# talmolab/track-mjx

Measured on AMD Instinct MI355X. Metric: env-steps/sec (whole node), rodent task @ 4096 envs/GPU, higher is better.
Workload: dtype f32

## Files before the change

### track_mjx_amd/csrc/wave_physics.h

```cpp
#pragma once
#include "tm_common.h"
#include "wave_layout.h"

#ifdef TM_HOST_EMU
#define TMW_NL 64
#define TMW_FOR for (int lane = 0; lane < 64; lane++)
#define TMW_SYNC() do { } while (0)
#define TMW_LI lane
#define TMW_LANE_DECL
#else
#define TMW_NL 1
#define TMW_FOR if (true)
#ifdef TMW_HARD_SYNC
#define TMW_SYNC() __syncthreads()
#else
#define TMW_SYNC() do { __builtin_amdgcn_fence(__ATOMIC_RELEASE, "wavefront"); __builtin_amdgcn_wave_barrier(); __builtin_amdgcn_fence(__ATOMIC_ACQUIRE, "wavefront"); } while (0)
#endif
#define TMW_LI 0
#define TMW_LANE_DECL const int lane = c.lane;
#endif
#define TMW_REG(type, name) type name[TMW_NL]
#ifdef TM_HOST_EMU
#define TMW_DUP_LANES_OK 0
#else
// ... 806 lines not shown
#pragma unroll
      for (int u = 0; u < 8; u++) {
        int mc = m0 + u < 64 ? m0 + u : 63;
        lm[u] = tmw_readlane(x, mc);
        ab[u] = tm_f2i(tmw_readlane(arow, mc));
      }
      TMW_FOR {
        float v[8]; int ad[8];
#pragma unroll
        for (int u = 0; u < 8; u++) ad[u] = lane > m0 + u ? ab[u] + lane : K.l_dummy + lane;
#pragma unroll
        for (int u = 0; u < 8; u++) v[u] = L[ad[u]];
        float s = acc[TMW_LI];
#pragma unroll
        for (int u = 0; u < 8; u++) s += lane > m0 + u ? lm[u] * v[u] : 0.f;
        acc[TMW_LI] = s;
      }
    }
    TMW_FOR { if (lane >= 1 && lane <= d) L[K.l_LD + ak + lane] = -acc[TMW_LI]; }
    TMW_SYNC();
  }
}
#define TMW_RL 63
TM_DEV float tmw_rcp(float x) {
#ifdef TM_HOST_EMU
  return 1.f / x;
#else
  float r = __builtin_amdgcn_rcpf(x);
  return fmaf(fmaf(-x, r, 1.f), r, r);
#endif
}
#ifdef TM_HOST_EMU
#define TMW_MASK(m64) (((((unsigned long long)(m64)) >> lane) & 1ull) != 0ull)
#define TMW_SCHED_FENCE() do { } while (0)
#define TMW_PIN(x) do { } while (0)
#else
TM_DEV unsigned long long tmw_lit64(unsigned long long m64) {
  unsigned hi = (unsigned)(m64 >> 32);
  asm("" : "+s"(hi));
  return ((unsigned long long)hi << 32) | (unsigned)m64;
}
#define TMW_MASK(m64) __builtin_amdgcn_inverse_ballot_w64((((unsigned long long)(m64)) >> 31) == 0x1ffffffffull ? tmw_lit64((unsigned long long)(m64)) : (unsigned long long)(m64))
#define TMW_PIN(x) asm volatile("" : "+v"(x))
#define TMW_SCHED_FENCE() __builtin_amdgcn_sched_barrier(0)
#endif
#define TMW_M_LT(n) ((n) >= 64 ? ~0ull : ((1ull << (n)) - 1ull))
#define TMW_M_EQ(n) (1ull << (n))
#define TMW_M_RANGE(a, b) (TMW_M_LT(b) & ~TMW_M_LT(a))
#ifdef TM_HOST_EMU
struct tmw_f2 { float x, y; };
TM_DEV tmw_f2 tmw_fnma2(float ax, float ay, float bx, float by, tmw_f2 c) { tmw_f2 r; r.x = c.x - ax * bx; r.y = c.y - ay * by; return r; }
#define TMW_PIN2(v) do { } while (0)
#else
typedef float tmw_f2 __attribute__((ext_vector_type(2)));
TM_DEV tmw_f2 tmw_fnma2(float ax, float ay, float bx, float by, tmw_f2 c) { tmw_f2 a = {ax, ay}, b = {bx, by}; return __builtin_elementwise_fma(-a, b, c); }
#define TMW_PIN2(v) asm volatile("" : "+v"(v))
#endif
#define TMW_ROW(arr, k) (((k) & 1) ? arr[(k) >> 1][TMW_LI].y : arr[(k) >> 1][TMW_LI].x)
#define TMW_SET_ROW(arr, k, v) do { if ((k) & 1) arr[(k) >> 1][TMW_LI].y = (v); else arr[(k) >> 1][TMW_LI].x = (v); } while (0)
template <typename F>
TM_DEV void tmw_rank1_rows(tmw_f2 (*T)[TMW_NL], const int CNT, const int BASE, const float *rs, const float *rk, F after_top) {
  const int top = (CNT - 1) / 2;
  float alo = tmw_readlane(rs, BASE + 2 * top), ahi = 2 * top + 1 < CNT ? tmw_readlane(rs, BASE + 2 * top + 1) : 0.f;
#pragma unroll
  for (int p = top; p >= 0; p--) {
    float nlo = 0.f, nhi = 0.f;
    if (p > 0) { nlo = tmw_readlane(rs, BASE + 2 * p - 2); nhi = tmw_readlane(rs, BASE + 2 * p - 1); }
    if (2 * p + 1 < CNT) {
      TMW_FOR { T[p][TMW_LI] = tmw_fnma2(alo, ahi, rk[TMW_LI], rk[TMW_LI], T[p][TMW_LI]); TMW_PIN2(T[p][TMW_LI]); }
    } else {
      TMW_FOR { T[p][TMW_LI].x -= alo * rk[TMW_LI]; TMW_PIN2(T[p][TMW_LI]); }
    }
    if (p == top) after_top();
    alo = nlo; ahi = nhi;
  }
}
template <int FIRST, int N, int D0, bool EULER, bool RHS = EULER>
TM_DEV void tmw_rows_load(WCtx &c, const WLayout &K, tmw_f2 (*r)[TMW_NL], float hdamp, int rhs) {
  TmwModel &m = *c.mp; float *L = c.L; TMW_LANE_DECL
  const int adr0 = K.l_M + tmw_chain_madr(FIRST);
  TMW_REG(float, hd);
  if (EULER) { TMW_FOR { bool mine = TMW_MASK(TMW_M_RANGE(D0, D0 + N)); hd[TMW_LI] = mine ? L[K.l_hdamp + (mine ? FIRST + lane - D0 : 0)] : 0.f; } }
  TMW_FOR {
#pragma unroll
    for (int k = 0; k < N; k++) {
      const int dk = D0 + k, off = k * D0 + k * (k - 1) / 2 + k;
      float v = L[adr0 - lane + (off + dk)];
      if (EULER) v += TMW_MASK(TMW_M_EQ(dk)) ? hd[TMW_LI] : 0.f;
      v = TMW_MASK(TMW_M_LT(dk + 1)) ? v : 0.f;
      TMW_SET_ROW(r, k, v);
    }
    if (N & 1) r[N >> 1][TMW_LI].y = 0.f;
  }
  if (RHS) {
    TMW_REG(float, rhsv);
    TMW_FOR { rhsv[TMW_LI] = L[rhs + FIRST + (lane < N ? lane : N - 1)]; }
#pragma unroll
    for (int k = 0; k < N; k++) {
      float sk = tmw_readlane(rhsv, k);
      TMW_FOR { if (TMW_MASK(TMW_M_EQ(TMW_RL))) TMW_SET_ROW(r, k, sk); }
    }
  }
}
#ifdef TMW_TRUNK_F32
typedef float tmw_acc_t;
#else
typedef double tmw_acc_t;
#endif
struct TmwSchur {
#ifdef TM_HOST_EMU
  tmw_acc_t C[16][16];
#elif defined(TMW_TRUNK_F32)
  float __attribute__((ext_vector_type(4))) c;
#else
  double __attribute__((ext_vector_type(4))) c;
#endif
  float qa[4][TMW_NL], qb[4][TMW_NL];
  float yt[TMW_NL];
};
#ifndef TM_HOST_EMU
TM_DEV float tmw_pack4(float x0, float x1, float x2, float x3) {
  auto s01 = __builtin_amdgcn_permlane16_swap(tm_f2i(x0), tm_f2i(x1), false, false);
  auto s23 = __builtin_amdgcn_permlane16_swap(tm_f2i(x2), tm_f2i(x3), false, false);
  auto p = __builtin_amdgcn_permlane32_swap(s01[0], s23[0], false, false);
  return tm_i2f(p[0]);
}
TM_DEV int tmw_row_to0(int x, const int blk) {
  if (blk == 1) return __builtin_amdgcn_permlane16_swap(x, 0, false, false)[1];
  if (blk >= 2) {
    x = __builtin_amdgcn_permlane32_swap(x, 0, false, false)[1];
    if (blk == 3) x = __builtin_amdgcn_permlane16_swap(x, 0, false, false)[1];
  }
  return x;
}
TM_DEV double tmw_row_to0_d(double x, const int blk) {
  long long b; __builtin_memcpy(&b, &x, 8);
  int lo = tmw_row_to0((int)(b & 0xffffffffll), blk), hi = tmw_row_to0((int)(b >> 32), blk);
  b = ((long long)hi << 32) | (unsigned)lo;
  __builtin_memcpy(&x, &b, 8);
  return x;
}
TM_DEV double tmw_readlane_d(const double *v, int src) {
  long long b; __builtin_memcpy(&b, v, 8);
  int lo = __builtin_amdgcn_readlane((int)(b & 0xffffffffll), src), hi = __builtin_amdgcn_readlane((int)(b >> 32), src);
  b = ((long long)hi << 32) | (unsigned)lo;
  double r; __builtin_memcpy(&r, &b, 8);
  return r;
}
TM_DEV double tmw_rcp_d(double x) { double r = (double)__builtin_amdgcn_rcpf((float)x); return __builtin_fma(__builtin_fma(-x, r, 1.0), r, r); }
#else
TM_DEV double tmw_readlane_d(const double *v, int src) { return v[src]; }
TM_DEV double tmw_rcp_d(double x) { return 1.0 / x; }
#endif
#ifdef TMW_TRUNK_F32
TM_DEV float tmw_acc_readlane(const float *v, int src) { return tmw_readlane(v, src); }
TM_DEV float tmw_acc_rcp(float x) { return tmw_rcp(x); }
TM_DEV float tmw_acc_fnma(float a, float b, float c) { return fmaf(-a, b, c); }
#else
TM_DEV double tmw_acc_readlane(const double *v, int src) { return tmw_readlane_d(v, src); }
TM_DEV double tmw_acc_rcp(double x) { return tmw_rcp_d(x); }
TM_DEV double tmw_acc_fnma(double a, double b, double c) { return __builtin_fma(-a, b, c); }
TM_DEV float tmw_acc_readlane(const float *v, int src) { return tmw_readlane(v, src); }
TM_DEV float tmw_acc_rcp(float x) { return tmw_rcp(x); }
TM_DEV float tmw_acc_fnma(float a, float b, float c) { return fmaf(-a, b, c); }
#endif
template <bool EULER>
TM_DEV void tmw_schur_init(WCtx &c, const WLayout &K, TmwSchur &S, tmw_f2 (*tr)[TMW_NL], int rhs) {
  float *L = c.L; TMW_LANE_DECL
#ifdef TM_HOST_EMU
  for (int i = 0; i < 16; i++) for (int j = 0; j < 16; j++) S.C[i][j] = (i < TMW_RODENT_TRUNK) ? -(tmw_acc_t)((i & 1) ? tr[i >> 1][j].y : tr[i >> 1][j].x) : (tmw_acc_t)0;
  for (int q = 0; q < 4; q++) for (int l = 0; l < 64; l++) S.qa[q][l] = S.qb[q][l] = 0.f;
#else
#define TMW_TRROW(i) ((i) < TMW_RODENT_TRUNK ? -(((i) & 1) ? tr[(i) >> 1][0].y : tr[(i) >> 1][0].x) : 0.f)
#ifdef TMW_TRUNK_F32
  S.c[0] = tmw_pack4(TMW_TRROW(0), TMW_TRROW(4), TMW_TRROW(8), TMW_TRROW(12));
  S.c[1] = tmw_pack4(TMW_TRROW(1), TMW_TRROW(5), TMW_TRROW(9), TMW_TRROW(13));
  S.c[2] = tmw_pack4(TMW_TRROW(2), TMW_TRROW(6), TMW_TRROW(10), TMW_TRROW(14));
  S.c[3] = tmw_pack4(TMW_TRROW(3), TMW_TRROW(7), TMW_TRROW(11), TMW_TRROW(15));
#else
  S.c[0] = (double)tmw_pack4(TMW_TRROW(0), TMW_TRROW(1), TMW_TRROW(2), TMW_TRROW(3));
  S.c[1] = (double)tmw_pack4(TMW_TRROW(4), TMW_TRROW(5), TMW_TRROW(6), TMW_TRROW(7));
  S.c[2] = (double)tmw_pack4(TMW_TRROW(8), TMW_TRROW(9), TMW_TRROW(10), TMW_TRROW(11));
  S.c[3] = 0.0;
#endif
#undef TMW_TRROW
  for (int q = 0; q < 4; q++) S.qa[q][0] = S.qb[q][0] = 0.f;
#endif
  TMW_FOR { S.yt[TMW_LI] = EULER ? -L[rhs + (lane < TMW_RODENT_TRUNK ? lane : 0)] : 0.f; }
}
TM_DEV void tmw_schur_flush(TmwSchur &S) {
#ifdef TM_HOST_EMU
  for (int q = 0; q < 4; q++) for (int i = 0; i < 16; i++) for (int j = 0; j < 16; j++) S.C[i][j] += (tmw_acc_t)S.qa[q][i] * (tmw_acc_t)S.qb[q][j];
  for (int q = 0; q < 4; q++) for (int l = 0; l < 64; l++) S.qa[q][l] = S.qb[q][l] = 0.f;
#else
  float A = tmw_pack4(S.qa[0][0], S.qa[1][0], S.qa[2][0], S.qa[3][0]), B = tmw_pack4(S.qb[0][0], S.qb[1][0], S.qb[2][0], S.qb[3][0]);
#ifdef TMW_TRUNK_F32
  S.c = __builtin_amdgcn_mfma_f32_16x16x4f32(A, B, S.c, 0, 0, 0);
#else
  S.c = __builtin_amdgcn_mfma_f64_16x16x4f64((double)A, (double)B, S.c, 0, 0, 0);
#endif
  for (int q = 0; q < 4; q++) S.qa[q][0] = S.qb[q][0] = 0.f;
#endif
}
template <bool EULER>
TM_DEV void tmw_schur_apply(WCtx &c, TmwSchur &S, tmw_acc_t (*t)[TMW_NL]) {
  TMW_LANE_DECL
#pragma unroll
  for (int i = 0; i < TMW_RODENT_TRUNK; i++) {
#ifdef TM_HOST_EMU
    TMW_FOR { tmw_acc_t v = 0; if (lane < 16) v = -S.C[i][lane]; if (EULER && lane == TMW_RL) v = -(tmw_acc_t)S.yt[i]; t[i][TMW_LI] = v; }
#else
#ifdef TMW_TRUNK_F32
    float x = tm_i2f(tmw_row_to0(tm_f2i(S.c[i & 3]), i / 4));
#else
    double x = tmw_row_to0_d(S.c[i / 4], i & 3);
#endif
    tmw_acc_t v = TMW_MASK(TMW_M_LT(16)) ? -x : (tmw_acc_t)0;
    if (EULER) { float y = tmw_readlane(S.yt, i); v = TMW_MASK(TMW_M_EQ(TMW_RL)) ? (tmw_acc_t)(-y) : v; }
    t[i][0] = v;
#endif
  }
}
template <bool EULER, typename AT>
TM_DEV void tmw_trunk_factor(WCtx &c, const WLayout &K, AT (*t)[TMW_NL], int rhs) {
  float *L = c.L; TMW_LANE_DECL
  constexpr int N = TMW_RODENT_TRUNK;
  TMW_REG(float, dv); TMW_REG(float, yv);
  AT rs[2][TMW_NL], inv[2];
  TMW_FOR { dv[TMW_LI] = 0.f; yv[TMW_LI] = 0.f; }
  inv[(N - 1) & 1] = tmw_acc_rcp(tmw_acc_readlane(t[N - 1], N - 1));
  TMW_FOR { rs[(N - 1) & 1][TMW_LI] = t[N - 1][TMW_LI] * inv[(N - 1) & 1]; }
#pragma unroll
  for (int k = N - 1; k >= 0; k--) {
    const int off = k * (k - 1) / 2 + k, b = k & 1;
    if (k > 0) {
      { const AT a = tmw_acc_readlane(rs[b], k - 1); TMW_FOR { t[k - 1][TMW_LI] = tmw_acc_fnma(a, t[k][TMW_LI], t[k - 1][TMW_LI]); } }
      inv[b ^ 1] = tmw_acc_rcp(tmw_acc_readlane(t[k - 1], k - 1));
      TMW_FOR { rs[b ^ 1][TMW_LI] = t[k - 1][TMW_LI] * inv[b ^ 1]; }
    }
#pragma unroll
    for (int i = k - 2; i >= 0; i--) { const AT a = tmw_acc_readlane(rs[b], i); TMW_FOR { t[i][TMW_LI] = tmw_acc_fnma(a, t[k][TMW_LI], t[i][TMW_LI]); } }
    float yk = 0.f;
    if (EULER) yk = (float)tmw_acc_readlane(t[k], TMW_RL);
    TMW_FOR {
      if (EULER) yv[TMW_LI] = TMW_MASK(TMW_M_EQ(k)) ? yk : yv[TMW_LI];
      if (k > 0 && TMW_MASK(TMW_M_LT(k))) L[K.l_LD - lane + (off + k)] = (float)rs[b][TMW_LI];
      dv[TMW_LI] = TMW_MASK(TMW_M_EQ(k)) ? (float)inv[b] : dv[TMW_LI];
    }
  }
  TMW_FOR {
    if (TMW_MASK(TMW_M_LT(N))) { L[K.l_Dinv + lane] = dv[TMW_LI]; if (EULER) L[rhs + lane] = yv[TMW_LI]; }
  }
}

template <int FIRST, int N, int D0, bool EULER>
TM_DEV void tmw_rows_factor(WCtx &c, const WLayout &K, tmw_f2 (*r)[TMW_NL], TmwSchur *S, int rhs) {
  float *L = c.L; TMW_LANE_DECL
  const int adr0 = K.l_LD + tmw_chain_madr(FIRST);
  constexpr int Q0 = D0 > 0 ? tmw_chain_rows_before(FIRST) : 0;
  float rs[2][TMW_NL], rk[2][TMW_NL], inv[2];
  TMW_REG(float, dv);
  TMW_REG(float, yv);
  TMW_FOR { yv[TMW_LI] = 0.f; rk[(N - 1) & 1][TMW_LI] = TMW_ROW(r, N - 1); }
  inv[(N - 1) & 1] = tmw_rcp(tmw_readlane(rk[(N - 1) & 1], D0 + N - 1));
  TMW_FOR { rs[(N - 1) & 1][TMW_LI] = rk[(N - 1) & 1][TMW_LI] * inv[(N - 1) & 1]; }
#pragma unroll
  for (int k = N - 1; k >= 0; k--) {
    const int dk = D0 + k, off = k * D0 + k * (k - 1) / 2 + k, b = k & 1;
    if (k > 0) {
      tmw_rank1_rows(r, k, D0, rs[b], rk[b], [&]() {
        TMW_FOR { rk[b ^ 1][TMW_LI] = TMW_ROW(r, k - 1); }
        inv[b ^ 1] = tmw_rcp(tmw_readlane(rk[b ^ 1], dk - 1));
        TMW_FOR { rs[b ^ 1][TMW_LI] = rk[b ^ 1][TMW_LI] * inv[b ^ 1]; TMW_PIN(rs[b ^ 1][TMW_LI]); }
      });
    }
    float yk = 0.f;
    if (EULER) { yk = tmw_readlane(rk[b], TMW_RL); TMW_FOR { yv[TMW_LI] = TMW_MASK(TMW_M_EQ(k)) ? yk : yv[TMW_LI]; } }
    if (D0 > 0) {
      const int slot = (Q0 + (N - 1 - k)) & 3;
      TMW_FOR {
        float a = D0 < 16 ? (TMW_MASK(TMW_M_LT(D0)) ? rs[b][TMW_LI] : 0.f) : rs[b][TMW_LI];
        S->qa[slot][TMW_LI] = a;
        S->qb[slot][TMW_LI] = D0 < 16 ? (TMW_MASK(TMW_M_LT(D0)) ? rk[b][TMW_LI] : 0.f) : rk[b][TMW_LI];
      }
      if (EULER) { TMW_FOR { S->yt[TMW_LI] += S->qa[slot][TMW_LI] * yk; } }
      if (slot == 3) tmw_schur_flush(*S);
    }
    TMW_FOR {
      if (dk > 0 && TMW_MASK(TMW_M_LT(dk))) L[adr0 - lane + (off + dk)] = rs[b][TMW_LI];
      dv[TMW_LI] = TMW_MASK(TMW_M_EQ(dk)) ? inv[b] : dv[TMW_LI];
    }
  }
  TMW_FOR {
    if (TMW_MASK(TMW_M_RANGE(D0, D0 + N))) L[K.l_Dinv + FIRST - D0 + lane] = dv[TMW_LI];
    if (EULER && TMW_MASK(TMW_M_LT(N))) L[rhs + FIRST + lane] = yv[TMW_LI];
  }
}
template <int FIRST, int N, int D0, bool EULER>
TM_DEV void tmw_chain_factor(WCtx &c, const WLayout &K, TmwSchur *S, float hdamp, int rhs) {
  tmw_f2 r[(N + 1) / 2][TMW_NL];
  tmw_rows_load<FIRST, N, D0, EULER>(c, K, r, hdamp, rhs);
  tmw_rows_factor<FIRST, N, D0, EULER>(c, K, r, S, rhs);
}
template <bool EULER>
TM_DEV void tmw_factor_chains(WCtx &c, const WLayout &K, float hdamp, int rhs) {
  TmwSchur S;
  {
    tmw_f2 tr[(TMW_RODENT_TRUNK + 1) / 2][TMW_NL];
    tmw_rows_load<0, TMW_RODENT_TRUNK, 0, EULER, false>(c, K, tr, hdamp, rhs);
    tmw_schur_init<EULER>(c, K, S, tr, rhs);
  }
#define TMW_X(first, n, d0) tmw_chain_factor<first, n, d0, EULER>(c, K, &S, hdamp, rhs);
  TMW_RODENT_LEAF_CHAINS(TMW_X)
#undef TMW_X
  tmw_schur_flush(S);
  tmw_acc_t t[TMW_RODENT_TRUNK][TMW_NL];
  tmw_schur_apply<EULER>(c, S, t);
#if defined(TMW_TRUNK_ELIM_F32) && !defined(TMW_TRUNK_F32)
  { float tf[TMW_RODENT_TRUNK][TMW_NL];
    TMW_FOR { for (int i = 0; i < TMW_RODENT_TRUNK; i++) tf[i][TMW_LI] = (float)t[i][TMW_LI]; }
    tmw_trunk_factor<EULER, float>(c, K, tf, rhs); }
#else
  tmw_trunk_factor<EULER, tmw_acc_t>(c, K, t, rhs);
#endif
  TMW_SYNC();
}
TM_DEV void tmw_rows_accum(tmw_f2 &acc, const tmw_f2 (*S)[TMW_NL], const int CNT, const int BASE, const float *l, int li) {
#pragma unroll
  for (int p = 0; 2 * p < CNT; p++) {
    float alo = tmw_readlane(l, BASE + 2 * p), ahi = 2 * p + 1 < CNT ? tmw_readlane(l, BASE + 2 * p + 1) : 0.f;
    acc = tmw_fnma2(alo, ahi, S[p][li].x, S[p][li].y, acc);
  }
}
template <int FIRST, int N, int D0>
TM_DEV void tmw_chain_trunk_products(WCtx &c, const WLayout &K, const float (*Bp)[TMW_NL], const tmw_f2 (*tn)[TMW_NL], float (*P)[TMW_NL]) {
  float *L = c.L; TMW_LANE_DECL
  const int adr0 = K.l_LD + tmw_chain_madr(FIRST);
#ifdef TM_HOST_EMU
  (void)Bp;
  for (int k = 0; k < N; k++)
    TMW_FOR {
      float s = 0.f;
      if (lane < D0) for (int j = 0; j < D0; j++) s += L[adr0 + k * D0 + k * (k - 1) / 2 + k + (D0 + k) - j] * ((j & 1) ? tn[j >> 1][lane].y : tn[j >> 1][lane].x);
      P[k][TMW_LI] = s;
    }
#else
  (void)tn;
  typedef float __attribute__((ext_vector_type(4))) f4;
#pragma unroll
  for (int k0 = 0; k0 < N; k0 += 16) {
    const int kq = k0 + (lane & 15), kk = lane >> 4;
    const bool rowok = kq < N;
    const int kc = rowok ? kq : N - 1;
    const int base = adr0 + kc * D0 + kc * (kc - 1) / 2 + kc + (D0 + kc) - kk;
    f4 acc = {0.f, 0.f, 0.f, 0.f};
#pragma unroll
    for (int m = 0; 4 * m < D0; m++) {
      float a = L[base - 4 * m];
      a = (rowok && 4 * m + kk < D0) ? a : 0.f;
      acc = __builtin_amdgcn_mfma_f32_16x16x4f32(a, Bp[m][0], acc, 0, 0, 0);
    }
#pragma unroll
    for (int i = 0; i < 16; i++) {
      if (k0 + i >= N) break;
      float x = acc[i & 3];
      if ((i >> 2) == 1) x = tm_i2f(__builtin_amdgcn_permlane16_swap(tm_f2i(x), 0, false, false)[1]);
      else if ((i >> 2) >= 2) {
        x = tm_i2f(__builtin_amdgcn_permlane32_swap(tm_f2i(x), 0, false, false)[1]);
        if ((i >> 2) == 3) x = tm_i2f(__builtin_amdgcn_permlane16_swap(tm_f2i(x), 0, false, false)[1]);
      }
      P[k0 + i][0] = TMW_MASK(TMW_M_LT(D0)) ? x : 0.f;
    }
  }
#endif
}
template <int FIRST, int N, int D0>
TM_DEV void tmw_rows_invert(WCtx &c, const WLayout &K, tmw_f2 (*n)[TMW_NL], tmw_f2 (*tn)[TMW_NL], const float (*Bp)[TMW_NL]) {
  float *L = c.L; TMW_LANE_DECL
  const int adr0 = K.l_LD + tmw_chain_madr(FIRST);
  float l[N][TMW_NL], P[D0 > 0 ? N : 1][TMW_NL];
  tmw_f2 acc[TMW_NL];
  TMW_FOR {
#pragma unroll
    for (int k = 0; k < N; k++) {
      const int dk = D0 + k, off = k * D0 + k * (k - 1) / 2 + k;
      float v = L[adr0 - lane + (off + dk)];
      l[k][TMW_LI] = TMW_MASK(TMW_M_LT(dk)) ? v : 0.f;
    }
#pragma unroll
    for (int p = 0; p < (N + 1) / 2; p++) { n[p][TMW_LI].x = 0.f; n[p][TMW_LI].y = 0.f; }
  }
  if (D0 > 0) tmw_chain_trunk_products<FIRST, N, D0>(c, K, Bp, tn, P);
#pragma unroll
  for (int k = 0; k < N; k++) {
    const int dk = D0 + k, off = k * D0 + k * (k - 1) / 2 + k;
    TMW_FOR { acc[TMW_LI].x = (TMW_MASK(TMW_M_EQ(dk)) ? 1.f : 0.f) - (D0 > 0 ? P[D0 > 0 ? k : 0][TMW_LI] : 0.f); acc[TMW_LI].y = 0.f; }
    if (k > 0) { TMW_FOR { tmw_rows_accum(acc[TMW_LI], n, k, D0, l[k], TMW_LI); } }
    TMW_FOR {
      float v = acc[TMW_LI].x + acc[TMW_LI].y;
      TMW_SET_ROW(n, k, v);
      if (TMW_MASK(TMW_M_LT(dk + 1))) L[adr0 - lane + (off + dk)] = v;
    }
  }
}
template <int FIRST, int N, int D0>
TM_DEV void tmw_chain_invert(WCtx &c, const WLayout &K, tmw_f2 (*tn)[TMW_NL], const float (*Bp)[TMW_NL]) {
  tmw_f2 n[(N + 1) / 2][TMW_NL];
  tmw_rows_invert<FIRST, N, D0>(c, K, n, tn, Bp);
}
TM_DEV void tmw_invert_chains(WCtx &c, const WLayout &K) {
  tmw_f2 tn[(TMW_RODENT_TRUNK + 1) / 2][TMW_NL];
  float Bp[(TMW_RODENT_TRUNK + 3) / 4][TMW_NL];
  tmw_rows_invert<0, TMW_RODENT_TRUNK, 0>(c, K, tn, tn, Bp);
#ifndef TM_HOST_EMU
#define TMW_TN(i) ((i) < TMW_RODENT_TRUNK ? (((i) & 1) ? tn[(i) >> 1][0].y : tn[(i) >> 1][0].x) : 0.f)
#pragma unroll
  for (int m = 0; m < (TMW_RODENT_TRUNK + 3) / 4; m++) Bp[m][0] = tmw_pack4(TMW_TN(4 * m), TMW_TN(4 * m + 1), TMW_TN(4 * m + 2), TMW_TN(4 * m + 3));
#undef TMW_TN
#endif
#define TMW_X(first, n, d0) tmw_chain_invert<first, n, d0>(c, K, tn, Bp);
  TMW_RODENT_LEAF_CHAINS(TMW_X)
#undef TMW_X
  TMW_SYNC();
}
template <int FIRST, int N, int D0>
TM_DEV void tmw_rows_subst(WCtx &c, const WLayout &K, const float *xt, float *z, int x) {
  float *L = c.L; TMW_LANE_DECL
  constexpr int QMAX = D0 + N - 1;
  TMW_REG(float, bv);
  TMW_FOR {
    int k = lane < N ? lane : N - 1;
    int base = K.l_LD + tmw_chain_madr(FIRST) + k * D0 + k * (k - 1) / 2 + k + D0 + k - QMAX;
    bv[TMW_LI] = tm_i2f(base);
    z[TMW_LI] = L[x + FIRST + k] * L[K.l_Dinv + FIRST + k];
  }
#pragma unroll
  for (int q = 0; q < D0; q++) {
    float xq = tmw_readlane(xt, q);
    TMW_FOR { z[TMW_LI] -= L[tm_f2i(bv[TMW_LI]) + (QMAX - q)] * xq; }
  }
#pragma unroll
  for (int q = D0; q < QMAX; q++) {
    float xq = tmw_readlane(z, q - D0);
    TMW_FOR { float v = L[tm_f2i(bv[TMW_LI]) + (QMAX - q)]; z[TMW_LI] = TMW_MASK(TMW_M_RANGE(q - D0 + 1, N)) ? z[TMW_LI] - v * xq : z[TMW_LI]; }
  }
  TMW_FOR { if (TMW_MASK(TMW_M_LT(N))) L[x + FIRST + lane] = z[TMW_LI]; }
}
TM_DEV void tmw_subst_chains(WCtx &c, const WLayout &K, int x) {
  TMW_LANE_DECL
  TMW_REG(float, xt); TMW_REG(float, z);
  TMW_FOR { xt[TMW_LI] = 0.f; }
  tmw_rows_subst<0, TMW_RODENT_TRUNK, 0>(c, K, xt, xt, x);
#define TMW_X(first, n, d0) tmw_rows_subst<first, n, d0>(c, K, xt, z, x);
  TMW_RODENT_LEAF_CHAINS(TMW_X)
#undef TMW_X
  TMW_SYNC();
}
template <int FIRST, int N, int D0>
TM_DEV void tmw_rows_colacc(WCtx &c, const WLayout &K, int A, const float *xv, float *acc) {
  float *L = c.L; TMW_LANE_DECL
  const int adr0 = A + tmw_chain_madr(FIRST);
#pragma unroll
  for (int k = N - 1; k >= 1 - (D0 > 0); k--) {
    const int dk = D0 + k, off = k * D0 + k * (k - 1) / 2 + k;
    float xk = tmw_readlane(xv, dk);
    TMW_FOR { float v = L[adr0 - lane + (off + dk)]; acc[TMW_LI] += (TMW_MASK(TMW_M_LT(dk)) ? v : 0.f) * xk; }
  }
}
template <bool SOLVE>
TM_DEV void tmw_colpart_chains(WCtx &c, const WLayout &K, int A, int x, int out) {
  float *L = c.L; TMW_LANE_DECL
  float xv[TMW_RODENT_NCHAIN + 1][TMW_NL], acc[TMW_RODENT_NCHAIN + 1][TMW_NL];
  { int ci = 0;
#define TMW_X(first, n, d0) TMW_FOR { bool mine = TMW_MASK(TMW_M_RANGE(d0, d0 + n)); xv[ci][TMW_LI] = mine ? L[x + (mine ? first - d0 + lane : 0)] : 0.f; acc[ci][TMW_LI] = 0.f; } ci++;
  TMW_RODENT_LEAF_CHAINS(TMW_X)
  TMW_X(0, TMW_RODENT_TRUNK, 0)
#undef TMW_X
  }
  { int ci = 0;
#define TMW_X(first, n, d0) tmw_rows_colacc<first, n, d0>(c, K, A, xv[ci], acc[ci]); TMW_FOR { acc[TMW_RODENT_NCHAIN][TMW_LI] += TMW_MASK(TMW_M_LT(d0)) ? acc[ci][TMW_LI] : 0.f; } ci++;
  TMW_RODENT_LEAF_CHAINS(TMW_X)
#undef TMW_X
  tmw_rows_colacc<0, TMW_RODENT_TRUNK, 0>(c, K, A, xv[ci], acc[ci]); }
  { int ci = 0;
#define TMW_STORE(first, n, d0) TMW_FOR { if (TMW_MASK(TMW_M_RANGE(d0, d0 + n))) { float v = acc[ci][TMW_LI]; if (SOLVE) v = (xv[ci][TMW_LI] + v) * L[K.l_Dinv + first - d0 + lane]; L[out + first - d0 + lane] = v; } } ci++;
  TMW_RODENT_LEAF_CHAINS(TMW_STORE)
  TMW_STORE(0, TMW_RODENT_TRUNK, 0)
#undef TMW_STORE
  }
  TMW_SYNC();
}
TM_DEV float tmw_row_dot(const float *L, const WLayout &K, int A, int x, int i, bool diag) {
  int w0 = tm_f2i(L[K.l_tdof + 2 * i]), w1 = tm_f2i(L[K.l_tdof + 2 * i + 1]);
  int d = TMW_DEPTH(w0), adr = TMW_ADR(w0), r = i - (w1 & 0xff), jp1 = (w1 >> 8) & 0xff;
  const float *Ap = L + A + adr, *xp = L + x;
  float acc = diag ? Ap[0] * xp[i] : 0.f;
#pragma unroll 4
  for (int q = 1; q <= r; q++) acc += Ap[q] * xp[i - q];
  const float *Aq = Ap + r + 1;
#pragma unroll 4
  for (int t = 0; t < d - r; t++) acc += Aq[t] * xp[jp1 - 1 - t];
  return acc;
}
TM_DEV float tmw_col_dot(const float *L, const WLayout &K, int A, int x, int i) {
  int w0 = tm_f2i(L[K.l_tdof + 2 * i]), nd = (tm_f2i(L[K.l_tdof + 2 * i + 1]) >> 16) & 0xff, d = TMW_DEPTH(w0);
  const float *Ap = L + A - d, *xp = L + x + i + 1;
  const float *tw = L + K.l_tdof + 2 * (i + 1);
  float acc = 0.f;
#pragma unroll 4
  for (int t = 0; t < nd; t++) acc += Ap[TMW_MEND(tm_f2i(tw[2 * t]))] * xp[t];
  return acc;
}
#ifdef TM_HOST_EMU
TM_DEV int tmw_opaque_s(int x) { return x; }
#else
TM_DEV int tmw_opaque_s(int x) { asm volatile("" : "+s"(x)); return x; }
#endif
template <int MAXR0, int MAXR1, int MAXT>
TM_DEV void tmw_row_runs2(const float *L, const WLayout &K, int A, int x, int lane, bool diag, float &z0, float &z1, int tp0, int tp1) {
  const int i0 = lane, i1 = lane + 64 < K.nv ? lane + 64 : 64;
  int d0, r0, j0, d1, r1, j1, adr0, adr1;
  if (K.lean) {
    d0 = TMW_TP_DEPTH(tp0); r0 = TMW_TP_RUN(tp0); j0 = d0 - r0; adr0 = TMW_TP_MEND(tp0) - d0;
    d1 = TMW_TP_DEPTH(tp1); r1 = TMW_TP_RUN(tp1); j1 = d1 - r1; adr1 = TMW_TP_MEND(tp1) - d1;
  } else {
    int w00 = tm_f2i(L[K.l_tdof + 2 * i0]), w01 = tm_f2i(L[K.l_tdof + 2 * i0 + 1]);
    int w10 = tm_f2i(L[K.l_tdof + 2 * i1]), w11 = tm_f2i(L[K.l_tdof + 2 * i1 + 1]);
    d0 = TMW_DEPTH(w00); r0 = i0 - (w01 & 0xff); j0 = (w01 >> 8) & 0xff; adr0 = TMW_ADR(w00);
    d1 = TMW_DEPTH(w10); r1 = i1 - (w11 & 0xff); j1 = (w11 >> 8) & 0xff; adr1 = TMW_ADR(w10);
  }
  const float *A0 = L + A + adr0, *x0 = L + x + i0, *A1 = L + A + adr1, *x1 = L + x + i1;
  float a0 = diag ? A0[0] * x0[0] : 0.f, a1 = diag ? A1[0] * x1[0] : 0.f;
  const int maxr0 = tmw_opaque_s(MAXR0), maxr1 = tmw_opaque_s(MAXR1), maxt = tmw_opaque_s(MAXT);
#pragma unroll 4
  for (int q = 1; q <= maxr1; q++) {
    float u0 = A0[q], v0 = x0[-q], u1 = A1[q], v1 = x1[-q];
    a0 = fmaf(q <= r0 ? u0 : 0.f, v0, a0); a1 = fmaf(q <= r1 ? u1 : 0.f, v1, a1);
  }
#pragma unroll 8
  for (int q = maxr1 + 1; q <= maxr0; q++) { float u0 = A0[q], v0 = x0[-q]; a0 = fmaf(q <= r0 ? u0 : 0.f, v0, a0); }
  const float *B0 = A0 + r0 + 1, *y0 = L + x + j0 - 1, *B1 = A1 + r1 + 1, *y1 = L + x + j1 - 1;
  const int n0 = d0 - r0, n1 = d1 - r1;
#pragma unroll 4
  for (int t = 0; t < maxt; t++) {
    float u0 = B0[t], v0 = y0[-t], u1 = B1[t], v1 = y1[-t];
    a0 = fmaf(t < n0 ? u0 : 0.f, v0, a0); a1 = fmaf(t < n1 ? u1 : 0.f, v1, a1);
  }
  z0 = a0; z1 = a1;
}
TM_DEV void tmw_rowpart_chains(WCtx &c, const WLayout &K, int A, int x, bool diag, float *z0, float *z1) {
  float *L = c.L; TMW_LANE_DECL
  TMW_FOR { tmw_row_runs2<tmw_chain_maxrun(0, 64), tmw_chain_maxrun(64, 73), TMW_RODENT_TRUNK>(L, K, A, x, lane, diag, z0[TMW_LI], z1[TMW_LI], tmw_opaque_v(c.tp0[TMW_LI]), tmw_opaque_v(c.tp1[TMW_LI])); }
}
TM_DEV void tmw_solve(WCtx &c, const WLayout &K, int x, int tmp) {
  float *L = c.L; TMW_LANE_DECL
  TMW_REG(float, z0); TMW_REG(float, z1);
  if (K.chains) {
    TMW_TICK2(15);
    tmw_colpart_chains<true>(c, K, K.l_LD, x, x);
    TMW_TICK2(26);
    tmw_rowpart_chains(c, K, K.l_LD, x, false, z0, z1);
    TMW_FOR { z0[TMW_LI] += L[x + lane]; if (lane + 64 < K.nv) z1[TMW_LI] += L[x + lane + 64]; }
    TMW_SYNC();
    TMW_FOR { L[x + lane] = z0[TMW_LI]; if (lane + 64 < K.nv) L[x + lane + 64] = z1[TMW_LI]; }
    TMW_SYNC();
    return;
  }
  TMW_FOR {
    for (int slot = 0; slot < 2; slot++) {
      int i = lane + 64 * slot;
      if (i >= K.nv) continue;
      (slot ? z1 : z0)[TMW_LI] = (L[x + i] + tmw_col_dot(L, K, K.l_LD, x, i)) * L[K.l_Dinv + i];
    }
  }
  TMW_SYNC();
  TMW_FOR {
    for (int slot = 0; slot < 2; slot++) { int i = lane + 64 * slot; if (i < K.nv) L[x + i] = (slot ? z1 : z0)[TMW_LI]; }
  }
  TMW_SYNC();
  TMW_FOR {
    for (int slot = 0; slot < 2; slot++) {
      int i = lane + 64 * slot;
      if (i >= K.nv) continue;
      (slot ? z1 : z0)[TMW_LI] = L[x + i] + tmw_row_dot(L, K, K.l_LD, x, i, false);
    }
  }
  TMW_SYNC();
  TMW_FOR {
    for (int slot = 0; slot < 2; slot++) { int i = lane + 64 * slot; if (i < K.nv) L[x + i] = (slot ? z1 : z0)[TMW_LI]; }
  }
  TMW_SYNC();
}
TM_DEV void tmw_mul_m(WCtx &c, const WLayout &K, int x, int y) {
  float *L = c.L; TMW_LANE_DECL
  if (K.chains) {
    TMW_REG(float, z0); TMW_REG(float, z1);
    TMW_TICK2(15);
    tmw_rowpart_chains(c, K, K.l_M, x, true, z0, z1);
    TMW_SCHED_FENCE();
    tmw_colpart_chains<false>(c, K, K.l_M, x, y);
    TMW_FOR { L[y + lane] += z0[TMW_LI]; if (lane + 64 < K.nv) L[y + lane + 64] += z1[TMW_LI]; }
    TMW_SYNC();
    TMW_TICK2(24);
  } else {
    TMW_FOR {
      for (int i = lane; i < K.nv; i += 64) L[y + i] = tmw_row_dot(L, K, K.l_M, x, i, true) + tmw_col_dot(L, K, K.l_M, x, i);
    }
    TMW_SYNC();
  }
}

TM_DEV void tmw_jmul_stage1(WCtx &c, const WLayout &K, int v) {
  TmwModel &m = *c.mp; float *L = c.L; TMW_LANE_DECL
  if (c.nact == c.nla) return;
  TMW_FOR {
    if (lane < K.ngroup * 6) {
      int g = lane / 6, k = lane - g * 6, ld, d, run, jp1;
      if (K.lean) { const int gp = tm_f2i(L[K.l_tgrp + g]); ld = (gp & 0xff) == 0xff ? -1 : (gp & 0xff); d = (gp >> 8) & 0xff; run = (gp >> 16) & 0xff; jp1 = d - run; }
      else { ld = ((const signed char *)(L + K.l_tgrp))[g]; const int w1 = TMW_W1(ld >= 0 ? ld : 0); d = TMW_DEPTH(TMW_W0(ld >= 0 ? ld : 0)); run = ld - (w1 & 0xff); jp1 = (w1 >> 8) & 0xff; }
      float s = 0.f;
      if (ld >= 0) {
#pragma unroll 4
        for (int q = 0; q <= d; q++) { int i = tmw_anc_r(ld, q, run, jp1); s += L[K.l_cdof + i * 6 + k] * L[v + i]; }
      }
      L[K.l_sv + lane] = s;
    }
  }
}
TM_DEV void tmw_jmul_stage2(WCtx &c, const WLayout &K, int v, int out) {
  TmwModel &m = *c.mp; float *L = c.L; TMW_LANE_DECL
  TMW_FOR {
    const unsigned char *rm = TMW_ROWMAP(K);
    for (int kr = lane; kr < c.nact; kr += 64) {
      int r = rm[kr];
      float o;
      if (kr < c.nla) {
        o = ((r & 0x80) ? -1.f : 1.f) * L[v + (r & 0x7f)];
      } else {
        int cc = (r - K.nlim) >> 2, e = (r - K.nlim) & 3;
        const float *sv = L + K.l_sv + TMW_CONGRP(K)[cc] * 6, *off = L + K.l_con_off + cc * 3;
        float fr[9];
        tmw_get_con_frame(L, K, cc, fr);
        tm_cross(fr + 6, fr, fr + 3);
        float cr[3], vel[3];
        tm_cross(cr, sv, off);
        for (int k = 0; k < 3; k++) vel[k] = sv[3 + k] + cr[k];
        float a0 = tm_dot3(fr, vel), at = tm_dot3(fr + 3 + 3 * (e >> 1), vel) * TMW_MU(cc);
        o = (e & 1) ? a0 - at : a0 + at;
      }
      L[out + kr] = o;
    }
  }
}
TM_DEV void tmw_jmul(WCtx &c, const WLayout &K, int v, int out) {
  tmw_jmul_stage1(c, K, v);
  TMW_SYNC();
  tmw_jmul_stage2(c, K, v, out);
  TMW_SYNC();
}
TM_DEV void tmw_jt_force(WCtx &c, const WLayout &K, int out) {
  TmwModel &m = *c.mp; float *L = c.L; TMW_LANE_DECL
  const bool anycon = c.nact > c.nla;
  if (anycon) {
  TMW_FOR {
    for (int cc = lane; cc < K.ncon; cc += 64) {
      const bool on = L[K.l_con_dist + cc] < 0.f;
      const int r0b = TMW_CCROW(K)[cc], r0 = on ? r0b : 0;
      float ja[4], D[4], f[4];
#pragma unroll
      for (int e = 0; e < 4; e++) { ja[e] = L[K.l_Jaref + r0 + e]; D[e] = L[K.l_efc_D + TMW_DIDX(r0 + e)]; }
      const float mu = TMW_MU(cc);
      const float *off = L + K.l_con_off + cc * 3;
      const float o0 = off[0], o1 = off[1], o2 = off[2];
      float fr[9];
      tmw_get_con_frame(L, K, cc, fr);
#pragma unroll
      for (int e = 0; e < 4; e++) f[e] = ja[e] < 0.f ? -D[e] * ja[e] : 0.f;
      float c0 = f[0] + f[1] + f[2] + f[3], c1 = mu * (f[0] - f[1]), c2 = mu * (f[2] - f[3]);
      tm_cross(fr + 6, fr, fr + 3);
      float F[3], T[3];
      const float ov[3] = {o0, o1, o2};
      for (int k = 0; k < 3; k++) F[k] = c0 * fr[k] + c1 * fr[3 + k] + c2 * fr[6 + k];
      tm_cross(T, ov, F);
      for (int k = 0; k < 3; k++) { L[K.l_wr + cc * 6 + k] = on ? T[k] : 0.f; L[K.l_wr + cc * 6 + 3 + k] = on ? F[k] : 0.f; }
    }
  }
  TMW_SYNC();
  TMW_REG(float, W0); TMW_REG(float, W1);
  TMW_FOR {
    for (int slot = 0; slot < 2; slot++) {
      int idx = lane + 64 * slot;
      float sacc = 0.f;
      if (idx < m.n_wsub * 6) {
        int su = idx / 6, k = idx - su * 6;
        unsigned m0 = slot == 0 && m.n_wsub * 6 <= 64 ? c.kmask[TMW_LI] : m.wsub_cmask[su][0], m1 = K.ncon > 32 ? m.wsub_cmask[su][1] : 0u;
        const unsigned char *rm = TMW_ROWMAP(K);
        for (int kr = c.nla; kr < c.nact; kr += 4) {
          int cc = (rm[kr] - K.nlim) >> 2;
          float w = L[K.l_wr + cc * 6 + k];
          bool in = ((cc < 32 ? m0 >> cc : m1 >> (cc - 32)) & 1u) != 0u;
          sacc += in ? w : 0.f;
        }
      }
      (slot ? W1 : W0)[TMW_LI] = sacc;
      if (m.n_wsub * 6 <= 64) break;
    }
  }
  TMW_SYNC();
  TMW_FOR {
    if (lane < m.n_wsub * 6) L[K.l_wr + lane] = W0[TMW_LI];
    if (lane + 64 < m.n_wsub * 6) L[K.l_wr + lane + 64] = W1[TMW_LI];
  }
  TMW_SYNC();
  }
  TMW_FOR {
    const bool ok1 = TMW_OK1(K);
    const int ii[2] = {lane, TMW_I1(K)};
    int sv[2], su[2], kr[2]; float s[2];
#pragma unroll
    for (int t = 0; t < 2; t++) {
      const int i = ii[t];
      const int lr = K.lean ? (i >= 6 ? i - 6 : -1) : TMW_LIMROW1(TMW_W0(i)) - 1;
      su[t] = K.lean ? TMW_TP_WSUB1(TMW_TP(lane + 64 * t)) - 1 : TMW_WSUB1(TMW_W1(i)) - 1;
      const int svb = TMW_LIMSIGN(K)[lr >= 0 ? lr : 0];
      sv[t] = lr >= 0 ? svb : 0;
    }
#pragma unroll
    for (int t = 0; t < 2; t++) kr[t] = sv[t] != 0 ? (sv[t] < 0 ? -sv[t] : sv[t]) - 1 : 0;
    const float ja0 = L[K.l_Jaref + kr[0]], D0 = L[K.l_efc_D + TMW_DIDX(kr[0])], ja1 = L[K.l_Jaref + kr[1]], D1 = L[K.l_efc_D + TMW_DIDX(kr[1])];
    { const float fl = -D0 * ja0; s[0] = (sv[0] != 0 && ja0 < 0.f) ? (sv[0] > 0 ? fl : -fl) : 0.f; }
    { const float fl = -D1 * ja1; s[1] = (sv[1] != 0 && ja1 < 0.f) ? (sv[1] > 0 ? fl : -fl) : 0.f; }
    if (anycon) {
      float cd[2][6], w[2][6];
#pragma unroll
      for (int t = 0; t < 2; t++) { const int sw = su[t] >= 0 ? su[t] : 0; for (int k = 0; k < 6; k++) { cd[t][k] = L[K.l_cdof + ii[t] * 6 + k]; w[t][k] = L[K.l_wr + sw * 6 + k]; } }
#pragma unroll
      for (int t = 0; t < 2; t++) { float a = s[t]; for (int k = 0; k < 6; k++) a += cd[t][k] * w[t][k]; s[t] = su[t] >= 0 ? a : s[t]; }
    }
    L[out + lane] = s[0]; if (ok1) L[out + ii[1]] = s[1];
  }
  TMW_SYNC();
}

TM_DEV void tmw_mul_m_jmul(WCtx &c, const WLayout &K, int x, int y, int out) {
  float *L = c.L; TMW_LANE_DECL
  if (!K.chains) { tmw_mul_m(c, K, x, y); tmw_jmul(c, K, x, out); return; }
  TMW_REG(float, z0); TMW_REG(float, z1);
  TMW_TICK2(15);
  tmw_jmul_stage1(c, K, x);
  tmw_rowpart_chains(c, K, K.l_M, x, true, z0, z1);
  TMW_SCHED_FENCE();
  tmw_colpart_chains<false>(c, K, K.l_M, x, y);
  tmw_jmul_stage2(c, K, x, out);
  TMW_FOR { L[y + lane] += z0[TMW_LI]; if (lane + 64 < K.nv) L[y + lane + 64] += z1[TMW_LI]; }
  TMW_SYNC();
  TMW_TICK2(24);
}

// ... 799 lines not shown
```

Baseline: 1.721 million.

## Interleave independent leaf-chain factor, invert and substitution steps for ILP

Leaf chains of the rodent kinematic tree used to be processed one after another in the factorization, inversion and forward-substitution phases. Now chains are paired, or all interleaved in the substitution, so their independent dependency chains overlap inside one wavefront, with LDS loads software-pipelined one step ahead. In the factor phase the longer chain's Schur rows are kept and replayed later so the accumulation order stays the same. This hides per-step latency (readlane, rcp, LDS reads) at the cost of more live registers, which could lower occupancy or cause spills.

```diff
diff --git a/track_mjx_amd/csrc/wave_physics.h b/track_mjx_amd/csrc/wave_physics.h
--- a/track_mjx_amd/csrc/wave_physics.h
+++ b/track_mjx_amd/csrc/wave_physics.h
@@ -1132,6 +1132,108 @@
   tmw_rows_load<FIRST, N, D0, EULER>(c, K, r, hdamp, rhs);
   tmw_rows_factor<FIRST, N, D0, EULER>(c, K, r, S, rhs);
 }
+#define TMW_RODENT_LEAF_PAIRS(X) X(65, 8, 6, 57, 8, 6) X(48, 9, 6, 24, 24, 12) X(18, 6, 12, 12, 6, 12)
+constexpr bool tmw_pairs_match_chains() {
+  int n = 0; bool ok = true;
+#define TMW_X(fa, na, da, fb, nb, db) ok = ok && tmw_chain_rows_before(fa) == n && tmw_chain_rows_before(fb) == n + na && tmw_chain_depth(fa) == da && tmw_chain_depth(fb) == db \
+    && tmw_chain_depth(fa + na - 1) == da + na - 1 && tmw_chain_depth(fb + nb - 1) == db + nb - 1; n += na + nb;
+  TMW_RODENT_LEAF_PAIRS(TMW_X)
+#undef TMW_X
+  return ok && n == tmw_chain_rows_before(-1);
+}
+constexpr int tmw_chain_index(int first) {
+  int n = 0;
+#define TMW_X(f, len, d0) if (f == first) return n; n++;
+  TMW_RODENT_LEAF_CHAINS(TMW_X)
+#undef TMW_X
+  return n;
+}
+template <int V> struct TmwConst { static constexpr int v = V; };
+static_assert(tmw_pairs_match_chains(), "TMW_RODENT_LEAF_PAIRS must list TMW_RODENT_LEAF_CHAINS two by two, in order");
+#ifndef TMW_CHAINS_SERIAL
+template <int N> struct TmwChainFac {
+  tmw_f2 r[(N + 1) / 2][TMW_NL];
+  float rs[2][TMW_NL], rk[2][TMW_NL], inv[2];
+  float dv[TMW_NL], yv[TMW_NL];
+};
+template <int N> struct TmwKeptRows { float a[N][TMW_NL], b[N][TMW_NL], y[N]; };
+template <int FIRST, int N, int D0>
+TM_DEV void tmw_fac_first_pivot(TmwChainFac<N> &F) {
+  TMW_FOR { F.yv[TMW_LI] = 0.f; F.rk[(N - 1) & 1][TMW_LI] = TMW_ROW(F.r, N - 1); }
+  F.inv[(N - 1) & 1] = tmw_rcp(tmw_readlane(F.rk[(N - 1) & 1], D0 + N - 1));
+  TMW_FOR { F.rs[(N - 1) & 1][TMW_LI] = F.rk[(N - 1) & 1][TMW_LI] * F.inv[(N - 1) & 1]; }
+}
+template <int FIRST, int N, int D0, bool EULER, bool KEEP, int NK>
+TM_DEV void tmw_fac_step(WCtx &c, const WLayout &K, TmwChainFac<N> &F, TmwSchur *S, TmwKeptRows<NK> &kept, const int k) {
+  float *L = c.L; TMW_LANE_DECL
+  const int adr0 = K.l_LD + tmw_chain_madr(FIRST);
+  constexpr int Q0 = tmw_chain_rows_before(FIRST);
+  const int dk = D0 + k, off = k * D0 + k * (k - 1) / 2 + k, b = k & 1;
+  if (k > 0) {
+    tmw_rank1_rows(F.r, k, D0, F.rs[b], F.rk[b], [&]() {
+      TMW_FOR { F.rk[b ^ 1][TMW_LI] = TMW_ROW(F.r, k - 1); }
+      F.inv[b ^ 1] = tmw_rcp(tmw_readlane(F.rk[b ^ 1], dk - 1));
+      TMW_FOR { F.rs[b ^ 1][TMW_LI] = F.rk[b ^ 1][TMW_LI] * F.inv[b ^ 1]; TMW_PIN(F.rs[b ^ 1][TMW_LI]); }
+    });
+  }
+  float yk = 0.f;
+  if (EULER) { yk = tmw_readlane(F.rk[b], TMW_RL); TMW_FOR { F.yv[TMW_LI] = TMW_MASK(TMW_M_EQ(k)) ? yk : F.yv[TMW_LI]; } }
+  if (KEEP) {
+    TMW_FOR {
+      kept.a[N - 1 - k][TMW_LI] = D0 < 16 ? (TMW_MASK(TMW_M_LT(D0)) ? F.rs[b][TMW_LI] : 0.f) : F.rs[b][TMW_LI];
+      kept.b[N - 1 - k][TMW_LI] = D0 < 16 ? (TMW_MASK(TMW_M_LT(D0)) ? F.rk[b][TMW_LI] : 0.f) : F.rk[b][TMW_LI];
+    }
+    kept.y[N - 1 - k] = yk;
+  } else {
+    const int slot = (Q0 + (N - 1 - k)) & 3;
+    TMW_FOR {
+      float a = D0 < 16 ? (TMW_MASK(TMW_M_LT(D0)) ? F.rs[b][TMW_LI] : 0.f) : F.rs[b][TMW_LI];
+      S->qa[slot][TMW_LI] = a;
+      S->qb[slot][TMW_LI] = D0 < 16 ? (TMW_MASK(TMW_M_LT(D0)) ? F.rk[b][TMW_LI] : 0.f) : F.rk[b][TMW_LI];
+    }
+    if (EULER) { TMW_FOR { S->yt[TMW_LI] += S->qa[slot][TMW_LI] * yk; } }
+    if (slot == 3) tmw_schur_flush(*S);
+  }
+  TMW_FOR {
+    if (dk > 0 && TMW_MASK(TMW_M_LT(dk))) L[adr0 - lane + (off + dk)] = F.rs[b][TMW_LI];
+    F.dv[TMW_LI] = TMW_MASK(TMW_M_EQ(dk)) ? F.inv[b] : F.dv[TMW_LI];
+  }
+}
+template <int FIRST, int N, int D0, bool EULER>
+TM_DEV void tmw_fac_store(WCtx &c, const WLayout &K, TmwChainFac<N> &F, int rhs) {
+  float *L = c.L; TMW_LANE_DECL
+  TMW_FOR {
+    if (TMW_MASK(TMW_M_RANGE(D0, D0 + N))) L[K.l_Dinv + FIRST - D0 + lane] = F.dv[TMW_LI];
+    if (EULER && TMW_MASK(TMW_M_LT(N))) L[rhs + FIRST + lane] = F.yv[TMW_LI];
+  }
+}
+template <int FA, int NA, int DA, int FB, int NB, int DB, bool EULER>
+TM_DEV void tmw_pair_factor(WCtx &c, const WLayout &K, TmwSchur *S, float hdamp, int rhs) {
+  static_assert(NA <= NB && DA > 0 && DB > 0 && tmw_chain_rows_before(FB) == tmw_chain_rows_before(FA) + NA, "a pair = two neighbours of the chain list, the shorter first");
+  TmwChainFac<NA> A; TmwChainFac<NB> B; TmwKeptRows<NA> kept, none;
+  tmw_rows_load<FA, NA, DA, EULER>(c, K, A.r, hdamp, rhs);
+  tmw_rows_load<FB, NB, DB, EULER>(c, K, B.r, hdamp, rhs);
+  tmw_fac_first_pivot<FA, NA, DA>(A);
+  tmw_fac_first_pivot<FB, NB, DB>(B);
+#pragma unroll
+  for (int s = 0; s < NA; s++) {
+    tmw_fac_step<FA, NA, DA, EULER, false>(c, K, A, S, none, NA - 1 - s);
+    tmw_fac_step<FB, NB, DB, EULER, true>(c, K, B, S, kept, NB - 1 - s);
+  }
+  tmw_fac_store<FA, NA, DA, EULER>(c, K, A, rhs);
+#pragma unroll
+  for (int s = 0; s < NA; s++) {
+    constexpr int QB = tmw_chain_rows_before(FB);
+    const int slot = (QB + s) & 3;
+    TMW_FOR { S->qa[slot][TMW_LI] = kept.a[s][TMW_LI]; S->qb[slot][TMW_LI] = kept.b[s][TMW_LI]; }
+    if (EULER) { TMW_FOR { S->yt[TMW_LI] += S->qa[slot][TMW_LI] * kept.y[s]; } }
+    if (slot == 3) tmw_schur_flush(*S);
+  }
+#pragma unroll
+  for (int s = NA; s < NB; s++) tmw_fac_step<FB, NB, DB, EULER, false>(c, K, B, S, none, NB - 1 - s);
+  tmw_fac_store<FB, NB, DB, EULER>(c, K, B, rhs);
+}
+#endif
 template <bool EULER>
 TM_DEV void tmw_factor_chains(WCtx &c, const WLayout &K, float hdamp, int rhs) {
   TmwSchur S;
@@ -1140,9 +1242,15 @@
     tmw_rows_load<0, TMW_RODENT_TRUNK, 0, EULER, false>(c, K, tr, hdamp, rhs);
     tmw_schur_init<EULER>(c, K, S, tr, rhs);
   }
+#ifdef TMW_CHAINS_SERIAL
 #define TMW_X(first, n, d0) tmw_chain_factor<first, n, d0, EULER>(c, K, &S, hdamp, rhs);
   TMW_RODENT_LEAF_CHAINS(TMW_X)
 #undef TMW_X
+#else
+#define TMW_X(fa, na, da, fb, nb, db) tmw_pair_factor<fa, na, da, fb, nb, db, EULER>(c, K, &S, hdamp, rhs);
+  TMW_RODENT_LEAF_PAIRS(TMW_X)
+#undef TMW_X
+#endif
   tmw_schur_flush(S);
   tmw_acc_t t[TMW_RODENT_TRUNK][TMW_NL];
   tmw_schur_apply<EULER>(c, S, t);
@@ -1238,6 +1346,51 @@
   tmw_f2 n[(N + 1) / 2][TMW_NL];
   tmw_rows_invert<FIRST, N, D0>(c, K, n, tn, Bp);
 }
+#ifndef TMW_CHAINS_SERIAL
+template <int FIRST, int N, int D0>
+TM_DEV void tmw_inv_begin(WCtx &c, const WLayout &K, tmw_f2 (*n)[TMW_NL], float (*l)[TMW_NL], float (*P)[TMW_NL], tmw_f2 (*tn)[TMW_NL], const float (*Bp)[TMW_NL]) {
+  float *L = c.L; TMW_LANE_DECL
+  const int adr0 = K.l_LD + tmw_chain_madr(FIRST);
+  TMW_FOR {
+#pragma unroll
+    for (int k = 0; k < N; k++) {
+      const int dk = D0 + k, off = k * D0 + k * (k - 1) / 2 + k;
+      float v = L[adr0 - lane + (off + dk)];
+      l[k][TMW_LI] = TMW_MASK(TMW_M_LT(dk)) ? v : 0.f;
+    }
+#pragma unroll
+    for (int p = 0; p < (N + 1) / 2; p++) { n[p][TMW_LI].x = 0.f; n[p][TMW_LI].y = 0.f; }
+  }
+  tmw_chain_trunk_products<FIRST, N, D0>(c, K, Bp, tn, P);
+}
+template <int FIRST, int N, int D0>
+TM_DEV void tmw_inv_row(WCtx &c, const WLayout &K, tmw_f2 (*n)[TMW_NL], const float (*l)[TMW_NL], const float (*P)[TMW_NL], const int k) {
+  float *L = c.L; TMW_LANE_DECL
+  const int adr0 = K.l_LD + tmw_chain_madr(FIRST);
+  tmw_f2 acc[TMW_NL];
+  const int dk = D0 + k, off = k * D0 + k * (k - 1) / 2 + k;
+  TMW_FOR { acc[TMW_LI].x = (TMW_MASK(TMW_M_EQ(dk)) ? 1.f : 0.f) - P[k][TMW_LI]; acc[TMW_LI].y = 0.f; }
+  if (k > 0) { TMW_FOR { tmw_rows_accum(acc[TMW_LI], n, k, D0, l[k], TMW_LI); } }
+  TMW_FOR {
+    float v = acc[TMW_LI].x + acc[TMW_LI].y;
+    TMW_SET_ROW(n, k, v);
+    if (TMW_MASK(TMW_M_LT(dk + 1))) L[adr0 - lane + (off + dk)] = v;
+  }
+}
+template <int FA, int NA, int DA, int FB, int NB, int DB>
+TM_DEV void tmw_pair_invert(WCtx &c, const WLayout &K, tmw_f2 (*tn)[TMW_NL], const float (*Bp)[TMW_NL]) {
+  static_assert(NA <= NB && DA > 0 && DB > 0, "leaf chains, the shorter first");
+  tmw_f2 nA[(NA + 1) / 2][TMW_NL], nB[(NB + 1) / 2][TMW_NL];
+  float lA[NA][TMW_NL], PA[NA][TMW_NL], lB[NB][TMW_NL], PB[NB][TMW_NL];
+  tmw_inv_begin<FA, NA, DA>(c, K, nA, lA, PA, tn, Bp);
+  tmw_inv_begin<FB, NB, DB>(c, K, nB, lB, PB, tn, Bp);
+#pragma unroll
+  for (int k = 0; k < NB; k++) {
+    if (k < NA) tmw_inv_row<FA, NA, DA>(c, K, nA, lA, PA, k);
+    tmw_inv_row<FB, NB, DB>(c, K, nB, lB, PB, k);
+  }
+}
+#endif
 TM_DEV void tmw_invert_chains(WCtx &c, const WLayout &K) {
   tmw_f2 tn[(TMW_RODENT_TRUNK + 1) / 2][TMW_NL];
   float Bp[(TMW_RODENT_TRUNK + 3) / 4][TMW_NL];
@@ -1248,9 +1401,15 @@
   for (int m = 0; m < (TMW_RODENT_TRUNK + 3) / 4; m++) Bp[m][0] = tmw_pack4(TMW_TN(4 * m), TMW_TN(4 * m + 1), TMW_TN(4 * m + 2), TMW_TN(4 * m + 3));
 #undef TMW_TN
 #endif
+#ifdef TMW_CHAINS_SERIAL
 #define TMW_X(first, n, d0) tmw_chain_invert<first, n, d0>(c, K, tn, Bp);
   TMW_RODENT_LEAF_CHAINS(TMW_X)
 #undef TMW_X
+#else
+#define TMW_X(fa, na, da, fb, nb, db) tmw_pair_invert<fa, na, da, fb, nb, db>(c, K, tn, Bp);
+  TMW_RODENT_LEAF_PAIRS(TMW_X)
+#undef TMW_X
+#endif
   TMW_SYNC();
 }
 template <int FIRST, int N, int D0>
@@ -1276,14 +1435,76 @@
   }
   TMW_FOR { if (TMW_MASK(TMW_M_LT(N))) L[x + FIRST + lane] = z[TMW_LI]; }
 }
+#ifndef TMW_CHAINS_SERIAL
+template <int FIRST, int N, int D0>
+TM_DEV void tmw_subst_begin(WCtx &c, const WLayout &K, float *bv, float *z, int x) {
+  float *L = c.L; TMW_LANE_DECL
+  constexpr int QMAX = D0 + N - 1;
+  TMW_FOR {
+    int k = lane < N ? lane : N - 1;
+    int base = K.l_LD + tmw_chain_madr(FIRST) + k * D0 + k * (k - 1) / 2 + k + D0 + k - QMAX;
+    bv[TMW_LI] = tm_i2f(base);
+    z[TMW_LI] = L[x + FIRST + k] * L[K.l_Dinv + FIRST + k];
+  }
+}
+template <int FIRST, int N, int D0>
+TM_DEV void tmw_subst_load(WCtx &c, const float *bv, float *v, const int q) {
+  float *L = c.L;
+  constexpr int QMAX = D0 + N - 1;
+  if (q < QMAX) { TMW_FOR { v[TMW_LI] = L[tm_f2i(bv[TMW_LI]) + (QMAX - q)]; } }
+}
+template <int FIRST, int N, int D0>
+TM_DEV void tmw_subst_term(WCtx &c, const float *xt, float *z, const float *v, const int q) {
+  TMW_LANE_DECL
+  constexpr int QMAX = D0 + N - 1;
+  if (q < D0) {
+    float xq = tmw_readlane(xt, q);
+    TMW_FOR { z[TMW_LI] -= v[TMW_LI] * xq; }
+  } else if (q < QMAX) {
+    float xq = tmw_readlane(z, q - D0);
+    TMW_FOR { z[TMW_LI] = TMW_MASK(TMW_M_RANGE(q - D0 + 1, N)) ? z[TMW_LI] - v[TMW_LI] * xq : z[TMW_LI]; }
+  }
+}
+template <int FIRST, int N, int D0>
+TM_DEV void tmw_subst_store(WCtx &c, const float *z, int x) {
+  float *L = c.L; TMW_LANE_DECL
+  TMW_FOR { if (TMW_MASK(TMW_M_LT(N))) L[x + FIRST + lane] = z[TMW_LI]; }
+}
+#endif
 TM_DEV void tmw_subst_chains(WCtx &c, const WLayout &K, int x) {
   TMW_LANE_DECL
-  TMW_REG(float, xt); TMW_REG(float, z);
+  TMW_REG(float, xt);
   TMW_FOR { xt[TMW_LI] = 0.f; }
   tmw_rows_subst<0, TMW_RODENT_TRUNK, 0>(c, K, xt, xt, x);
+#ifdef TMW_CHAINS_SERIAL
+  TMW_REG(float, z);
 #define TMW_X(first, n, d0) tmw_rows_subst<first, n, d0>(c, K, xt, z, x);
   TMW_RODENT_LEAF_CHAINS(TMW_X)
 #undef TMW_X
+#else
+  constexpr int QALL = tmw_chain_maxdepth(TMW_RODENT_TRUNK, 73);
+#define TMW_CI(first) (TmwConst<tmw_chain_index(first)>::v)
+  float bv[TMW_RODENT_NCHAIN][TMW_NL], z[TMW_RODENT_NCHAIN][TMW_NL], v[2][TMW_RODENT_NCHAIN][TMW_NL];
+#define TMW_X(first, n, d0) tmw_subst_begin<first, n, d0>(c, K, bv[TMW_CI(first)], z[TMW_CI(first)], x);
+  TMW_RODENT_LEAF_CHAINS(TMW_X)
+#undef TMW_X
+#define TMW_X(first, n, d0) tmw_subst_load<first, n, d0>(c, bv[TMW_CI(first)], v[0][TMW_CI(first)], 0);
+  TMW_RODENT_LEAF_CHAINS(TMW_X)
+#undef TMW_X
+#pragma unroll
+  for (int q = 0; q < QALL; q++) {
+#define TMW_X(first, n, d0) tmw_subst_load<first, n, d0>(c, bv[TMW_CI(first)], v[(q + 1) & 1][TMW_CI(first)], q + 1);
+    TMW_RODENT_LEAF_CHAINS(TMW_X)
+#undef TMW_X
+#define TMW_X(first, n, d0) tmw_subst_term<first, n, d0>(c, xt, z[TMW_CI(first)], v[q & 1][TMW_CI(first)], q);
+    TMW_RODENT_LEAF_CHAINS(TMW_X)
+#undef TMW_X
+  }
+#define TMW_X(first, n, d0) tmw_subst_store<first, n, d0>(c, z[TMW_CI(first)], x);
+  TMW_RODENT_LEAF_CHAINS(TMW_X)
+#undef TMW_X
+#undef TMW_CI
+#endif
   TMW_SYNC();
 }
 template <int FIRST, int N, int D0>
```

After: 1.725 million (median of 6 runs). No clear change (+0.2%).
